# enricobottazzi/zk-fhe

Measured on AMD Instinct MI355X. Metric: BFV proofs/sec (k=13), higher is better.
Workload: dtype u32x8 (256-bit Montgomery integers over BN254 Fr/Fq)

## Files before the change

### zk-fhe_amd/csrc/core.hip

```cpp
#include <atomic>
#include <cstdio>
#include <cstdlib>
#include <cstring>

#include <map>
#include <mutex>
#include <utility>

#include "ctx.hpp"
#include "fq29.hip.hpp"
#include "fr29.hip.hpp"
#include "fr9.hip.hpp"

using namespace zk;

static thread_local std::string g_create_err;

int zk_fail(zkfhe_ctx *ctx, int code, const char *what, hipError_t e, const char *file, int line) {
  char buf[512];
  snprintf(buf, sizeof(buf), "%s failed: %s (%s:%d)", what, hipGetErrorString(e), file, line);
  if (ctx) ctx->err = buf; else g_create_err = buf;
  return code;
}
int zk_fail_msg(zkfhe_ctx *ctx, int code, const std::string &msg) {
// ... 11 lines not shown
  have = bytes;
  return ZKFHE_OK;
}

int zk_scratch(zkfhe_ctx *ctx, int slot, size_t bytes, void **out) {
  if (ctx->scratch_sz[slot] < bytes) {
    if (ctx->scratch[slot]) {
      ZK_HIP(ctx, hipStreamSynchronize(ctx->stream));
      ZK_HIP(ctx, hipFree(ctx->scratch[slot]));
      ctx->scratch[slot] = nullptr;
      ctx->scratch_sz[slot] = 0;
    }
    size_t want = bytes + bytes / 4;
    ZK_HIP(ctx, hipMalloc(&ctx->scratch[slot], want));
    ctx->scratch_sz[slot] = want;
  }
  *out = ctx->scratch[slot];
  return ZKFHE_OK;
}

Fr zk_fr_from_u64(uint64_t v) {
  Fr t = Fr::zero();
  t.l[0] = (u32)v;
  t.l[1] = (u32)(v >> 32);
  return fp_to_mont<FrP>(t);
}

Fr zk_fr_root_of_unity(int log_n) {
  Fr c;
  const u32 w[8] = {0x60c37c9cu, 0xd34f1ed9u, 0xd39329c8u, 0x3215cf6du, 0x3dd31f74u, 0x98865ea9u, 0x166d18b7u, 0x03ddb9f5u};
  for (int i = 0; i < 8; ++i) c.l[i] = w[i];
  Fr r = fp_to_mont<FrP>(c);
  for (int i = 0; i < 28 - log_n; ++i) r = fp_sqr<FrP>(r);
  return r;
}

__global__ void __launch_bounds__(256) k_copy16(const uint4 *__restrict__ src, uint4 *__restrict__ dst, size_t n16) {
  for (size_t i = blockIdx.x * (size_t)blockDim.x + threadIdx.x; i < n16; i += (size_t)gridDim.x * blockDim.x) dst[i] = src[i];
}
int zk_copy_d2d(zkfhe_ctx *ctx, void *dst, const void *src, size_t bytes) {
  if (!bytes) return ZKFHE_OK;
  if (bytes >= ((size_t)1 << 20) && (bytes & 15) == 0 && ((uintptr_t)dst & 15) == 0 && ((uintptr_t)src & 15) == 0) {
    const size_t n16 = bytes / 16;
    size_t blocks = (n16 + 255) / 256;
    const size_t cap = (size_t)ctx->num_cu * 32;
    k_copy16<<<(unsigned)(blocks > cap ? cap : blocks), 256, 0, ctx->stream>>>((const uint4 *)src, (uint4 *)dst, n16);
    ZK_LAUNCH_CHECK(ctx);
    return ZKFHE_OK;
  }
  ZK_HIP(ctx, zk_memcpy_async(ctx, dst, src, bytes, hipMemcpyDeviceToDevice, ctx->stream));
  return ZKFHE_OK;
}

extern "C" {

const char *zkfhe_version(void) { return "zkfhe-mi355x 0.1 (gfx950)"; }

int zkfhe_ctx_create(int device_id, void *hip_stream, zkfhe_ctx **out) {
  setenv("GPU_MAX_HW_QUEUES", "2", 0);
  if (!getenv("ZKFHE_SPIN_WAIT")) {
    (void)hipSetDevice(device_id);
    (void)hipSetDeviceFlags(hipDeviceScheduleBlockingSync);
    (void)hipGetLastError();
  }
  if (!out) return zk_fail_msg(nullptr, ZKFHE_EINVAL, "out is NULL");
  *out = nullptr;
  int count = 0;
  hipError_t e = hipGetDeviceCount(&count);
  if (e != hipSuccess || count == 0)
    return zk_fail_msg(nullptr, ZKFHE_ENODEV, std::string("no HIP device: ") + hipGetErrorString(e));
  if (device_id < 0 || device_id >= count) return zk_fail_msg(nullptr, ZKFHE_EINVAL, "device_id out of range");
  hipDeviceProp_t prop;
  ZK_HIP(nullptr, hipGetDeviceProperties(&prop, device_id));
  if (strncmp(prop.gcnArchName, "gfx950", 6) != 0)
    return zk_fail_msg(nullptr, ZKFHE_ENODEV, std::string("device is ") + prop.gcnArchName + ", this library is built for gfx950 only");
  ZK_HIP(nullptr, hipSetDevice(device_id));
  zkfhe_ctx *ctx = new zkfhe_ctx();
  static std::atomic<uint64_t> next_uid{1};
  ctx->uid = next_uid.fetch_add(1);
  ctx->device = device_id;
  ctx->num_cu = prop.multiProcessorCount;
  const char *chain_env = getenv("ZKFHE_CHAIN");
  ctx->chain_serial = chain_env && !strcmp(chain_env, "serial");
  const char *profile_env = getenv("ZKFHE_PROFILE");
  ctx->throughput = profile_env && !strcmp(profile_env, "throughput");
  if (hip_stream) {
    ctx->stream = (hipStream_t)hip_stream;
  } else {
    e = hipStreamCreateWithFlags(&ctx->stream, hipStreamNonBlocking);
    if (e != hipSuccess) { delete ctx; return zk_fail(nullptr, ZKFHE_EHIP, "hipStreamCreate", e, __FILE__, __LINE__); }
    ctx->own_stream = true;
  }
  if (hipHostMalloc(&ctx->bounce, zkfhe_ctx::BOUNCE_BYTES, hipHostMallocDefault) != hipSuccess) ctx->bounce = nullptr;
  if (hipEventCreateWithFlags(&ctx->wait_ev, hipEventBlockingSync | hipEventDisableTiming) != hipSuccess) ctx->wait_ev = nullptr;
  hipEventCreate(&ctx->ev0);
  hipEventCreate(&ctx->ev1);
  hipEventCreate(&ctx->pe0);
  hipEventCreate(&ctx->pe1);
  *out = ctx;
  return ZKFHE_OK;
}

int zkfhe_ctx_destroy(zkfhe_ctx *ctx) {
  ZK_ENTER(ctx);
  if (!ctx) return ZKFHE_OK;
  hipSetDevice(ctx->device);
  hipStreamSynchronize(ctx->stream);
  if (ctx->bounce) (void)hipHostFree(ctx->bounce);
  for (auto &kv : ctx->domains) {
    hipFree(kv.second.fwd);
    hipFree(kv.second.inv);
    hipFree(kv.second.fwd29);
    hipFree(kv.second.inv29);
    hipFree(kv.second.n_inv29_dev);
  }
  for (auto &kv : ctx->tw13) hipFree(kv.second);
  for (auto &kv : ctx->pre13) hipFree(kv.second);
  for (auto &kv : ctx->dif8) hipFree(kv.second);
  for (int i = 0; i < 4; ++i)
    if (ctx->scratch[i]) hipFree(ctx->scratch[i]);
  if (ctx->tickets) hipFree(ctx->tickets);
  if (ctx->bfv_tw) hipFree(ctx->bfv_tw);
  if (ctx->bfv_work) hipFree(ctx->bfv_work);
  for (auto &kv : ctx->slot_tw) hipFree(kv.second.dev);
  if (ctx->wait_ev) hipEventDestroy(ctx->wait_ev);
  hipEventDestroy(ctx->ev0);
  hipEventDestroy(ctx->ev1);
  if (ctx->own_stream) hipStreamDestroy(ctx->stream);
  delete ctx;
  return ZKFHE_OK;
}

const char *zkfhe_last_error(const zkfhe_ctx *ctx) { return ctx ? ctx->err.c_str() : g_create_err.c_str(); }

int zkfhe_sync(zkfhe_ctx *ctx) {
  ZK_ENTER(ctx);
  ZK_HIP(ctx, zk_wait(ctx));
  return ZKFHE_OK;
}

void *zkfhe_stream(zkfhe_ctx *ctx) { return (void *)ctx->stream; }

int zkfhe_device_info(zkfhe_ctx *ctx, char *arch_name, size_t arch_len, int *num_cu, size_t *hbm_bytes) {
  ZK_ENTER(ctx);
  hipDeviceProp_t prop;
  ZK_HIP(ctx, hipGetDeviceProperties(&prop, ctx->device));
  if (arch_name && arch_len) { strncpy(arch_name, prop.gcnArchName, arch_len - 1); arch_name[arch_len - 1] = 0; }
  if (num_cu) *num_cu = prop.multiProcessorCount;
  if (hbm_bytes) *hbm_bytes = prop.totalGlobalMem;
  return ZKFHE_OK;
}

int zkfhe_dev_alloc(zkfhe_ctx *ctx, size_t bytes, void **dptr) {
  ZK_ENTER(ctx);
  ZK_ARG(ctx, dptr != nullptr);
  ZK_HIP(ctx, hipSetDevice(ctx->device));
  hipError_t e = hipMalloc(dptr, bytes ? bytes : 1);
  if (e == hipErrorOutOfMemory) return zk_fail_msg(ctx, ZKFHE_ENOMEM, "hipMalloc: out of device memory");
  ZK_HIP(ctx, e);
  return ZKFHE_OK;
}
int zkfhe_dev_free(zkfhe_ctx *ctx, void *dptr) {
  ZK_ENTER(ctx);
  if (!dptr) return ZKFHE_OK;
  if (!ctx) {
    (void)hipFree(dptr);
// ... 300 lines not shown
```

### zk-fhe_amd/csrc/ctx.hpp

```cpp
#pragma once
#include <hip/hip_runtime.h>

#include <array>
#include <map>
#include <string>
#include <vector>

#include "../../include/zkfhe.h"
#include "bn254.hip.hpp"

struct NttDomain {
  int log_n = 0;
  zk::Fr *fwd = nullptr;
  zk::Fr *inv = nullptr;
  zk::Fr n_inv;
  zk::Fr omega, omega_inv;
  zk::Fr *fwd29 = nullptr, *inv29 = nullptr;
  zk::Fr n_inv29;
  zk::Fr *n_inv29_dev = nullptr;
};

struct zkfhe_ctx {
  uint64_t uid = 0;
  int device = 0;
  hipStream_t stream = nullptr;
  bool own_stream = false;
  hipEvent_t ev0 = nullptr, ev1 = nullptr;
  std::string err;
  int num_cu = 0;
  std::map<int, NttDomain> domains;
  std::map<const void *, void *> tw13;
  std::map<std::array<uint64_t, 6>, void *> pre13;
  std::map<std::array<uint64_t, 8>, void *> dif8;
  bool prof_on = false;
  hipEvent_t pe0 = nullptr, pe1 = nullptr;
  hipEvent_t wait_ev = nullptr;
  static constexpr int PROF_SLOTS = 28;
  double prof_ms[PROF_SLOTS] = {}, prof_bytes[PROF_SLOTS] = {}, prof_ops[PROF_SLOTS] = {};
  uint64_t prof_launches[PROF_SLOTS] = {};
  void *bounce = nullptr;
  static constexpr size_t BOUNCE_BYTES = (size_t)1 << 20;
  void *scratch[4] = {nullptr, nullptr, nullptr, nullptr};
  size_t scratch_sz[4] = {0, 0, 0, 0};
  float proof_marks[3] = {0, 0, 0};
  uint64_t cmd_count[3] = {0, 0, 0};
  zkfhe_ctx *cmd_owner = nullptr;
  bool chain_serial = false;
  bool throughput = false;
  unsigned *tickets = nullptr;
  uint32_t *bfv_tw = nullptr;
  void *bfv_work = nullptr;
  size_t bfv_work_sz = 0;
  struct SlotTables {
    uint32_t *dev = nullptr;
    uint32_t pinv = 0, n_inv = 0;
  };
  std::map<std::pair<uint64_t, uint64_t>, SlotTables> slot_tw;
};

struct zkfhe_basis {
  size_t n = 0;
  int c = 0;
  int windows = 0;
  zk::G1Affine *table = nullptr;
  zk::G1Affine *mult = nullptr;
  int mc = 0, mw = 0;
  size_t mult_bytes = 0;
  bool narrowed = false;
};

int zk_fail(zkfhe_ctx *ctx, int code, const char *what, hipError_t e, const char *file, int line);
int zk_fail_msg(zkfhe_ctx *ctx, int code, const std::string &msg);

#define ZK_HIP(ctx, expr)                                                             \
  do {                                                                                \
    hipError_t _e = (expr);                                                           \
    if (_e != hipSuccess) return zk_fail((ctx), ZKFHE_EHIP, #expr, _e, __FILE__, __LINE__); \
  } while (0)

enum { ZK_CMD_KERNEL = 0, ZK_CMD_COPY = 1, ZK_CMD_FILL = 2 };
static inline void zk_count(zkfhe_ctx *ctx, int which) { ++(ctx->cmd_owner ? ctx->cmd_owner : ctx)->cmd_count[which]; }

#define ZK_LAUNCH_CHECK(ctx)         \
  do {                               \
    zk_count((ctx), ZK_CMD_KERNEL);  \
    ZK_HIP(ctx, hipGetLastError());  \
  } while (0)

static inline hipError_t zk_memcpy_async(zkfhe_ctx *ctx, void *dst, const void *src, size_t bytes, hipMemcpyKind kind, hipStream_t stream) {
  zk_count(ctx, ZK_CMD_COPY);
  return hipMemcpyAsync(dst, src, bytes, kind, stream);
}
static inline hipError_t zk_memset_async(zkfhe_ctx *ctx, void *dst, int value, size_t bytes, hipStream_t stream) {
  zk_count(ctx, ZK_CMD_FILL);
  return hipMemsetAsync(dst, value, bytes, stream);
}

#define ZK_ENTER(ctx)                                   \
  do {                                                  \
    if (ctx) (void)hipSetDevice((ctx)->device);         \
  } while (0)

#define ZK_ARG(ctx, cond)                                                        \
  do {                                                                           \
    if (!(cond)) return zk_fail_msg((ctx), ZKFHE_EINVAL, std::string("bad argument: ") + #cond); \
  } while (0)

inline void zk_prof_begin(zkfhe_ctx *ctx) {
  if (ctx->prof_on) (void)hipEventRecord(ctx->pe0, ctx->stream);
}
inline void zk_prof_end(zkfhe_ctx *ctx, int which, double bytes) {
  if (!ctx->prof_on) return;
  (void)hipEventRecord(ctx->pe1, ctx->stream);
  (void)hipEventSynchronize(ctx->pe1);
  float ms = 0;
  (void)hipEventElapsedTime(&ms, ctx->pe0, ctx->pe1);
  ctx->prof_ms[which] += ms;
  ctx->prof_bytes[which] += bytes;
  ctx->prof_launches[which] += 1;
}

inline hipError_t zk_wait(zkfhe_ctx *ctx) {
  static const bool spin = getenv("ZKFHE_SPIN_WAIT") != nullptr;
  if (spin || !ctx->wait_ev) return hipStreamSynchronize(ctx->stream);
  hipError_t e = hipEventRecord(ctx->wait_ev, ctx->stream);
  if (e != hipSuccess) return e;
  return hipEventSynchronize(ctx->wait_ev);
}

int zk_dif8_pass(zkfhe_ctx *ctx, const zk::Fr *src, zk::Fr *dst, size_t n_cols, int log_n, int S, int inverse, const zk::Fr *shifts_host, unsigned rows);
int zk_msm_batch_strided(zkfhe_ctx *ctx, const zkfhe_basis *basis, const zkfhe_fr *scalars_dev, size_t col_stride, size_t n_cols, zkfhe_g1_affine *out_dev);
int zk_msm_batch_strided_form(zkfhe_ctx *ctx, const zkfhe_basis *basis, const zkfhe_fr *scalars_dev, size_t col_stride, size_t n_cols, void *out_dev, bool xyzz);
// ... 21 lines not shown
```

### zk-fhe_amd/csrc/msm.hip

```cpp
#include <algorithm>
#include <cstdio>
#include <cstring>
#include <vector>

#include "ctx.hpp"
#include "msm_plan.hpp"
#include "msm_sort.hip.hpp"
#include "msm_bucket.hip.hpp"
#include "msm_table.hip.hpp"

using namespace zk;

namespace {

constexpr size_t MSM_MAX_COLS = 4096;

__global__ void __launch_bounds__(256) k_g1_add(const G1Affine *__restrict__ a, const G1Affine *__restrict__ b,
                                                G1Affine *__restrict__ out, size_t n) {
  const size_t i = blockIdx.x * (size_t)blockDim.x + threadIdx.x;
  if (i >= n) return;
  G1X acc = g1x_from_affine(a[i]);
  g1x_add_affine(acc, b[i], false);
  out[i] = g1x_to_affine(acc);
}

__global__ void __launch_bounds__(256) k_g1_mul(const G1Affine *__restrict__ p, const Fr *__restrict__ k,
                                                G1Affine *__restrict__ out, size_t n) {
  const size_t i = blockIdx.x * (size_t)blockDim.x + threadIdx.x;
  if (i >= n) return;
  const Fr s = fp_from_mont<FrP>(k[i]);
  const G1Affine base = p[i];
  G1X acc = G1X::identity();
  for (int bit = 255; bit >= 0; --bit) {
    acc = g1x_dbl(acc);
    if ((s.l[bit >> 5] >> (bit & 31)) & 1) g1x_add_affine(acc, base, false);
  }
  out[i] = g1x_to_affine(acc);
}

int table_bits(size_t n, double budget_scale) {
  const char *e = getenv("ZKFHE_TABLE_BITS");
  const int forced = e ? atoi(e) : -1;
  const char *g = getenv("ZKFHE_TABLE_GB");
  double gb = g ? atof(g) : 48.0;
  if (!g) {
    size_t free_b = 0, total_b = 0;
    if (hipMemGetInfo(&free_b, &total_b) == hipSuccess && (double)free_b / 4.0 < gb * 1073741824.0) gb = (double)free_b / 4.0 / 1073741824.0;
  }
  const double budget = gb * 1073741824.0 * budget_scale;
  auto fits = [&](int c) {
    const double entries = (double)n * (double)((255 + c - 1) / c) * (double)(1u << (c - 1));
    return c >= 8 && c <= 15 && entries * sizeof(G1Affine) <= budget;
  };
  if (forced >= 0) return forced > 0 && fits(forced) ? forced : 0;
  for (int c = 15; c >= 8; --c)
    if (fits(c)) return c;
  return 0;
}

size_t table_reserve_bytes(size_t total_b) {
  if (const char *r = getenv("ZKFHE_TABLE_RESERVE_GB")) return (size_t)(atof(r) * 1073741824.0);
  const size_t eighth = total_b / 8, floor_b = (size_t)24 << 30;
  return eighth > floor_b ? eighth : floor_b;
}

BiasArg table_bias(int c, int W) {
  BiasArg B;
  memset(&B, 0, sizeof(B));
  for (int w = 0; w < W; ++w) {
    const int bit = c * w + c - 1;
    B.l[bit >> 5] |= 1u << (bit & 31);
  }
  return B;
}

int msm_table(zkfhe_ctx *ctx, const zkfhe_basis *basis, const Fr *scalars, size_t col_stride, size_t n_cols, void *out, bool xyzz) {
  const size_t n = basis->n;
  const int c = basis->mc, W = basis->mw;
  const size_t words = 2 * MSM_MAX_COLS + 4;
  if (!ctx->tickets) {
    ZK_HIP(ctx, hipMalloc((void **)&ctx->tickets, words * sizeof(unsigned)));
    ZK_HIP(ctx, zk_memset_async(ctx, ctx->tickets, 0, words * sizeof(unsigned), ctx->stream));
  }
  unsigned *n_part = ctx->tickets, *col_next = ctx->tickets + MSM_MAX_COLS;
  unsigned long long *adds = (unsigned long long *)(ctx->tickets + 2 * MSM_MAX_COLS);
  const size_t grid_max = (size_t)ctx->num_cu * 3;
#ifndef ZK_MSM_THROUGHPUT_P
#define ZK_MSM_THROUGHPUT_P 256
#endif
  size_t P = 256;
  const size_t P_min = ctx->throughput ? ZK_MSM_THROUGHPUT_P : 128;
  while (P > P_min && n_cols * ((n + P - 1) / P) < grid_max) P >>= 1;
  const size_t cpc = (n + P - 1) / P, n_items = n_cols * cpc;
  const size_t grid = n_items < grid_max ? n_items : grid_max;
  const size_t max_part = cpc < grid ? cpc : grid;
  const bool tree = n_cols <= 16;
  const unsigned L = tree ? 1 : 256;
  void *p0, *p1;
  ZK_CK(zk_scratch(ctx, 0, n_cols * max_part * L * sizeof(G1X), &p0));
  ZK_CK(zk_scratch(ctx, 1, grid * P * (size_t)W * 4, &p1));
  const int slot = n_cols * n > ((size_t)1 << 16) ? 0 : 2;
  if (ctx->prof_on) ZK_HIP(ctx, zk_memset_async(ctx, adds, 0, 8, ctx->stream));
  zk_prof_begin(ctx);
  (tree ? k_msm_table<true> : k_msm_table<false>)<<<(unsigned)grid, 256, 0, ctx->stream>>>(scalars, col_stride, n, basis->mult, c, W, table_bias(c, W), (unsigned)P, (unsigned)cpc,
                                                                                           (unsigned)n_cols, (unsigned)max_part, (G1X *)p0, n_part, col_next, (unsigned *)p1,
                                                                                           ctx->prof_on ? adds : nullptr);
  ZK_LAUNCH_CHECK(ctx);
  zk_prof_end(ctx, slot, 96.0 * (double)n * (double)n_cols);
  (xyzz ? k_msm_table_fold<true> : k_msm_table_fold<false>)<<<(unsigned)n_cols, 512, 0, ctx->stream>>>((const G1X *)p0, (unsigned)max_part, L, n_part, col_next, out);
  ZK_LAUNCH_CHECK(ctx);
  if (ctx->prof_on) {
    unsigned long long h = 0;
    ZK_HIP(ctx, hipMemcpy(&h, adds, 8, hipMemcpyDeviceToHost));
    ctx->prof_ops[slot] += (double)h;
  }
  return ZKFHE_OK;
}

int default_window_bits(size_t n) {
  if (n <= 64) return 5;
  if (n <= 1024) return 8;
  if (n <= 4096) return 11;
  if (n <= 16384) return 13;
  if (n <= 131072) return 14;
  return 16;
}

bool table_wide(const zkfhe_basis *b) {
  static const char *env = getenv("ZKFHE_TABLE_WIDE");
  return env ? env[0] == '1' : b->mw <= b->windows + 2;
}

static_assert(sizeof(G1X) == MSM_POINT_BYTES, "msm_plan.hpp sizes buckets, partials and marginals as G1X");
struct MsmScratch {
  char *p[MSM_ARRAYS];
  template <class T = unsigned>
  T *at(MsmArray a) const { return (T *)p[a]; }
};

int msm_scratch(zkfhe_ctx *ctx, const MsmGeometry &g, MsmScratch &a) {
  const MsmLayout l = msm_layout(g);
  void *slot[3];
  for (int s : {1, 2, 0}) ZK_CK(zk_scratch(ctx, s, l.slot_bytes[s], &slot[s]));
  for (int i = 0; i < MSM_ARRAYS; ++i) a.p[i] = (char *)slot[l.at[i].slot] + l.at[i].off;
  return ZKFHE_OK;
}

int sort_one_pass(zkfhe_ctx *ctx, const MsmGeometry &g, const MsmScratch &a, const Fr *scalars, size_t col_stride) {
  const unsigned gc = std::min(zk_blocks(g.n_cols * g.K1, 256), (unsigned)ctx->num_cu * 8);
  k_msm_clear<<<gc, 256, 0, ctx->stream>>>(a.at(HIST), g.n_cols * g.K1, a.at(HEAVY_COUNT));
  ZK_LAUNCH_CHECK(ctx);
  const unsigned chunks_per_col = (unsigned)((g.n + SORT_CHUNK - 1) / SORT_CHUNK);
  const unsigned grid = (unsigned)(g.n_cols * chunks_per_col);
  const size_t sort_lds = (size_t)g.K1 * sizeof(unsigned);
  if (sort_lds > 48 * 1024) {
    ZK_CK(zk_func_max_lds(ctx, (const void *)k_msm_hist, 160 * 1024));
    ZK_CK(zk_func_max_lds(ctx, (const void *)k_msm_scatter, 160 * 1024));
  }
  k_msm_hist<<<grid, SORT_THREADS, sort_lds, ctx->stream>>>(scalars, col_stride, g.n, chunks_per_col, g.c, g.W, a.at(HIST), g.K1);
  ZK_LAUNCH_CHECK(ctx);
  k_msm_scan<<<(unsigned)g.n_cols, 256, 0, ctx->stream>>>(a.at(HIST), a.at(OFF), a.at(CURSOR), g.K1);
  ZK_LAUNCH_CHECK(ctx);
  k_msm_scatter<<<grid, SORT_THREADS, sort_lds, ctx->stream>>>(scalars, col_stride, g.n, chunks_per_col, g.c, g.W, a.at(CURSOR), g.K1, a.at(ENTRIES), g.col_entries);
  ZK_LAUNCH_CHECK(ctx);
  return ZKFHE_OK;
}

int sort_two_level(zkfhe_ctx *ctx, const MsmGeometry &g, const MsmScratch &a, const Fr *scalars, size_t col_stride) {
  k_msm_clear<<<zk_blocks(g.n_cols * g.NB, 256), 256, 0, ctx->stream>>>(a.at(CHIST), g.n_cols * g.NB, a.at(HEAVY_COUNT));
  ZK_LAUNCH_CHECK(ctx);
  const unsigned ch_chunks = (unsigned)((g.n + CH_SCALARS - 1) / CH_SCALARS), cs_chunks = (unsigned)((g.n + CS_SCALARS - 1) / CS_SCALARS);
  k_msm_chist<<<(unsigned)(g.n_cols * ch_chunks), CS_THREADS, g.NB * sizeof(unsigned), ctx->stream>>>(scalars, col_stride, g.n, ch_chunks, g.c, g.W, g.L, g.NB, a.at(CHIST));
  ZK_LAUNCH_CHECK(ctx);
  k_msm_cscan<<<zk_blocks(g.n_cols, 64), 64, 0, ctx->stream>>>(a.at(CHIST), g.NB, g.n_cols, a.at(COFF), a.at(CCURSOR));
  ZK_LAUNCH_CHECK(ctx);
  const size_t cs_lds = ((size_t)3 * g.NB + (size_t)CS_SCALARS * g.W) * sizeof(unsigned);
  if (cs_lds > 48 * 1024) ZK_CK(zk_func_max_lds(ctx, (const void *)k_msm_cscatter, 64 * 1024));
  k_msm_cscatter<<<(unsigned)(g.n_cols * cs_chunks), CS_THREADS, cs_lds, ctx->stream>>>(scalars, col_stride, g.n, cs_chunks, g.c, g.W, g.L, g.NB, a.at(CCURSOR), a.at(STAGE),
                                                                                         g.stage_stride);
  ZK_LAUNCH_CHECK(ctx);
  ZK_CK(zk_func_max_lds(ctx, (const void *)k_msm_fine, (int)(FINE_TILE * sizeof(unsigned))));
  k_msm_fine<<<(unsigned)(g.n_cols * g.NB), FINE_THREADS, FINE_TILE * sizeof(unsigned), ctx->stream>>>(a.at(COFF), g.NB, g.L, a.at(STAGE), g.stage_stride, g.col_entries, g.K1,
                                                                                                        a.at(OFF), a.at(ENTRIES));
  ZK_LAUNCH_CHECK(ctx);
  return ZKFHE_OK;
}

int task_list(zkfhe_ctx *ctx, const MsmGeometry &g, const MsmScratch &a) {
  k_msm_task_count<<<(unsigned)g.n_cols, 256, 0, ctx->stream>>>(a.at(OFF), g.K, g.TASK_E, a.at(COL_HIST));
  ZK_LAUNCH_CHECK(ctx);
  k_msm_task_colscan<<<1, 128, 0, ctx->stream>>>(a.at(COL_HIST), (unsigned)g.n_cols, a.at(COL_BASE), a.at(N_TASKS));
  ZK_LAUNCH_CHECK(ctx);
  k_msm_task_fill<<<(unsigned)g.n_cols, 256, 0, ctx->stream>>>(a.at(OFF), g.K, g.TASK_E, a.at(COL_BASE), a.at(BUCKET_POS_A), a.at(BUCKET_POS_B), a.at<uint2>(TASKS),
// ... 216 lines not shown
```

### zk-fhe_amd/csrc/msm_table.hip.hpp

```cpp
#pragma once
#include "ctx.hpp"
#include "g1x29_wave.hip.hpp"

namespace {
using namespace zk;

struct BiasArg {
  u32 l[9];
};

__device__ __forceinline__ u32 bits_at(const u32 (&l)[9], int bit, int c) {
  const int limb = bit >> 5, sh = bit & 31;
  u32 lo = 0, hi = 0;
#pragma unroll
  for (int k = 0; k < 9; ++k) {
    if (k == limb) lo = l[k];
    if (k == limb + 1) hi = l[k];
  }
  return (u32)((((u64)hi << 32) | lo) >> sh) & ((1u << c) - 1);
}

__device__ __forceinline__ bool biased_scalar(const Fr &mont, const BiasArg &B, u32 (&out)[9], int &bits) {
  Fr s = fp_from_mont<FrP>(mont);
  const bool neg = fr_gt_half(s);
  if (neg) s = fp_neg<FrP>(s);
  bits = 0;
#pragma unroll
  for (int k = 0; k < 8; ++k)
    if (s.l[k]) bits = 32 * k + 32 - __clz(s.l[k]);
  u32 carry = 0;
#pragma unroll
  for (int k = 0; k < 8; ++k) {
    const u64 v = (u64)s.l[k] + B.l[k] + carry;
    out[k] = (u32)v;
    carry = (u32)(v >> 32);
  }
  out[8] = B.l[8] + carry;
  return neg;
}

__global__ void __launch_bounds__(64) k_basis_multiples(const G1Affine *__restrict__ bases, size_t n, int c, int W, G1Affine *__restrict__ T) {
  const size_t t = blockIdx.x * (size_t)blockDim.x + threadIdx.x;
  if (t >= n * (size_t)W) return;
  const size_t i = t / (size_t)W;
  const int w = (int)(t % (size_t)W);
  const size_t J = (size_t)1 << (c - 1);
  G1Affine *row = T + t * J;
  G1Affine b = bases[i];
  if (!b.is_identity() && w) b = g1x_to_affine(g1x_mul_pow2(g1x_from_affine(b), c * w));
  if (b.is_identity()) {
    for (size_t j = 0; j < J; ++j) row[j] = b;
    return;
  }
  row[0] = g1_affine_to_29(b);
  if (J == 1) return;
  G1X acc = g1x_from_affine_dbl(b);
  row[1] = g1_affine_to_29(g1x_to_affine(acc));
  for (size_t j = 2; j < J; ++j) {
    g1x_add_affine(acc, b, false);
    row[j] = g1_affine_to_29(g1x_to_affine(acc));
  }
}

template <bool TREE>
__global__ void __launch_bounds__(256, TREE ? 1 : 3) k_msm_table(const Fr *__restrict__ scalars, size_t col_stride, size_t n, const G1Affine *__restrict__ T, int c, int W, BiasArg B,
                                                   unsigned P, unsigned cpc , unsigned n_cols, unsigned max_part,
                                                   G1X *__restrict__ partials ,
                                                   unsigned *__restrict__ n_part ,
                                                   unsigned *__restrict__ col_next ,
                                                   unsigned *__restrict__ lists , unsigned long long *__restrict__ adds) {
  unsigned *__restrict__ lst = lists + (size_t)blockIdx.x * P * (unsigned)W;
  __shared__ G1X sh[TREE ? 128 : 1];
  __shared__ unsigned wave_cnt[4], item_sh;
  const unsigned lane = threadIdx.x & 63, wv = threadIdx.x >> 6;
  const int half = 1 << (c - 1);
  G1X29 acc = G1X29::identity();
  unsigned col = (unsigned)(((unsigned long long)blockIdx.x * n_cols) / gridDim.x), done = 0, total = 0;
  for (;;) {
    __syncthreads();
    if (threadIdx.x == 0) item_sh = atomicAdd(&col_next[col], 1u);
    __syncthreads();
    const unsigned chunk = item_sh;
    if (chunk >= cpc) {
      if (done) {
        if (TREE) acc = block_sum_256(acc, sh);
        __syncthreads();
        if (threadIdx.x == 0) item_sh = atomicAdd(&n_part[col], 1u);
        __syncthreads();
        const size_t slot = (size_t)col * max_part + item_sh;
        if (TREE) {
          if (threadIdx.x == 0) partials[slot] = g1x29_store(acc);
        } else {
          partials[slot * 256 + threadIdx.x] = g1x29_store(acc);
        }
        acc = G1X29::identity();
        done = 0;
      }
      __syncthreads();
      if (threadIdx.x == 0) item_sh = 0;
      __syncthreads();
      const unsigned MIN_JOIN = cpc < 4u ? cpc : 4u;
      unsigned best = 0;
      for (unsigned j = threadIdx.x; j < n_cols; j += 256) {
        const unsigned nx = __hip_atomic_load(&col_next[j], __ATOMIC_RELAXED, __HIP_MEMORY_SCOPE_AGENT);
        if (nx < cpc && (nx == 0 || cpc - nx >= MIN_JOIN)) {
          const unsigned h = ((j * 2654435761u) ^ (blockIdx.x * 40503u + 12345u) * 2246822519u) >> 13;
          best = max(best, (((h & 0x7ffffu) + 1u) << 12) | j);
        }
      }
      if (best) atomicMax(&item_sh, best);
      __syncthreads();
      const unsigned found = item_sh;
      if (!found) break;
      col = found & 4095u;
      continue;
    }
    ++done;
    {
      const size_t i = (size_t)chunk * P + threadIdx.x;
      const bool valid = threadIdx.x < P && i < n;
      u32 sb[9];
      bool neg = false;
      unsigned long long mask = 0;
      if (valid) {
        int bits;
        neg = biased_scalar(scalars[(size_t)col * col_stride + i], B, sb, bits);
        const int wtop = min(W, bits / c + 2);
        for (int w = 0; w < wtop; ++w)
          if ((int)bits_at(sb, w * c, c) != half) mask |= 1ull << w;
      }
      const unsigned mine = (unsigned)__popcll(mask);
      unsigned incl = mine;
#pragma unroll
      for (int d = 1; d < 64; d <<= 1) {
        const unsigned t = __shfl_up(incl, d);
        if ((int)lane >= d) incl += t;
      }
      if (lane == 63) wave_cnt[wv] = incl;
      __syncthreads();
      unsigned off = incl - mine;
      for (unsigned v = 0; v < wv; ++v) off += wave_cnt[v];
      const unsigned row0 = threadIdx.x * (unsigned)W;
      while (mask) {
        const int w = __builtin_ctzll(mask);
        mask &= mask - 1;
        const int d = (int)bits_at(sb, w * c, c) - half;
        lst[off++] = (((row0 + (unsigned)w) << (c - 1)) + (unsigned)(d < 0 ? -d : d) - 1u) | ((neg != (d < 0)) ? 0x80000000u : 0u);
      }
    }
    __syncthreads();
    const unsigned M = wave_cnt[0] + wave_cnt[1] + wave_cnt[2] + wave_cnt[3];
    total += M;
    const G1Affine *__restrict__ Tc = T + (((size_t)chunk * P * (size_t)W) << (c - 1));
    unsigned e = threadIdx.x, en = 0, en2 = 0;
    G1Affine p;
    if (e < M) {
      en = lst[e];
      p = Tc[en & 0x7fffffffu];
    }
    if (e + 256 < M) en2 = lst[e + 256];
    while (e < M) {
      const unsigned e2 = e + 256;
      unsigned en3 = 0;
      G1Affine p2;
      if (e2 < M) p2 = Tc[en2 & 0x7fffffffu];
      if (e2 + 256 < M) en3 = lst[e2 + 256];
      g1x29_add_affine(acc, g1a29_load(p), (en >> 31) != 0);
      e = e2;
      en = en2;
      en2 = en3;
      p = p2;
    }
  }
  if (adds && threadIdx.x == 0 && total) atomicAdd(adds, (unsigned long long)total);
}

template <bool XYZZ>
__global__ void __launch_bounds__(512) k_msm_table_fold(const G1X *__restrict__ partials, unsigned max_part, unsigned L, unsigned *__restrict__ n_part,
                                                        unsigned *__restrict__ col_next, void *__restrict__ out) {
  __shared__ G1X sh[256];
  const unsigned col = blockIdx.x, t = threadIdx.x & 255u, q = threadIdx.x >> 8;
  const unsigned np = n_part[col] * L;
  const G1X *mine = partials + (size_t)col * max_part * L;
  G1X29 f = G1X29::identity();
  {
    const unsigned first = L == 256 ? q * 256u + t : threadIdx.x, step = 512u;
    unsigned b = first;
    G1X cur;
    if (b < np) cur = mine[b];
    while (b < np) {
      const unsigned nb = b + step;
      G1X nxt;
      if (nb < np) nxt = mine[nb];
      g1x29_add(f, g1x29_load(cur));
      cur = nxt;
      b = nb;
    }
  }
  if (q == 1) sh[t] = g1x29_store(f);
  __syncthreads();
  if (q == 0) g1x29_add(f, g1x29_load(sh[t]));
  __syncthreads();
  if (q == 0 && t >= 128) sh[t - 128] = g1x29_store(f);
  __syncthreads();
  if (q == 0 && t < 128) g1x29_add(f, g1x29_load(sh[t]));
  __syncthreads();
  if (q == 0 && t >= 64 && t < 128) sh[t - 64] = g1x29_store(f);
  __syncthreads();
  if (threadIdx.x < 64) {
    g1x29_add(f, g1x29_load(sh[t]));
    for (int m = 1; m < 64; m <<= 1) {
      const G1X29 other = g1x_shfl_xor(f, m);
      g1x29_add(f, other);
    }
    if (threadIdx.x == 0) {
      if (XYZZ) ((G1X *)out)[col] = g1x29_to_std(f);
      else ((G1Affine *)out)[col] = g1x_to_affine(g1x29_to_std(f));
      n_part[col] = 0;
      col_next[col] = 0;
    }
  }
}

__global__ void __launch_bounds__(256) k_basis_table(const G1Affine *__restrict__ bases, size_t n, int c, int windows,
                                                     G1Affine *__restrict__ table) {
  const size_t i = blockIdx.x * (size_t)blockDim.x + threadIdx.x;
  if (i >= n) return;
  G1Affine p = bases[i];
  table[i] = g1_affine_to_29(p);
  G1X cur = g1x_from_affine(p);
  for (int w = 1; w < windows; ++w) {
    cur = g1x_mul_pow2(cur, c);
    G1Affine a = g1x_to_affine(cur);
    table[(size_t)w * n + i] = g1_affine_to_29(a);
    cur = g1x_from_affine(a);
  }
}

template <bool XYZZ>
__global__ void __launch_bounds__(64) k_msm_sparse(const zkfhe_sparse_term *__restrict__ terms, unsigned n_terms, const G1Affine *__restrict__ T, int c, int W,
                                                   BiasArg B, void *__restrict__ out) {
  const unsigned slot = blockIdx.x, lane = threadIdx.x;
  const int half = 1 << (c - 1);
  G1X29 acc = G1X29::identity();
  for (unsigned t = 0; t < n_terms; ++t) {
    if (terms[t].slot != slot) continue;
    Fr s;
#pragma unroll
    for (int i = 0; i < 4; ++i) {
      s.l[2 * i] = (u32)terms[t].scalar.l[i];
      s.l[2 * i + 1] = (u32)(terms[t].scalar.l[i] >> 32);
    }
    u32 sb[9];
    int bits;
    const bool neg = biased_scalar(s, B, sb, bits);
    const int d = (int)lane < W ? (int)bits_at(sb, (int)lane * c, c) - half : 0;
    if (d) {
// ... 16 lines not shown
```

### zk-fhe_amd/host/prove.hip

```cpp
#include "prover_internal.hpp"

int alloc_witness_buffers(zkfhe_ctx *ctx, const zkfhe_bfv_pk *pk, Workspace *ws) {
  if (ws->stream.p) return ZKFHE_OK;
  const size_t N = pk->prm.N;
  CK(ws->stream.alloc(ctx, (pk->gate1_cells + 8) * 32));
  CK(ws->pool.alloc(ctx, 40 * (2 * N + 8) * 32));
  CK(ws->invtmp.alloc(ctx, (pk->n_inv_slots + 8) * 32));
  ZK_HIP(ctx, hipHostMalloc((void **)&ws->host_pool, 24 * (2 * N + 8) * 32, hipHostMallocDefault));
  ws->host_poly_len = 2 * N + 8;
  ZK_HIP(ctx, hipHostMalloc((void **)&ws->host_poly, ws->host_poly_len * 32, hipHostMallocDefault));
  CK(ws->wblind.alloc(ctx, 256));
  ZK_HIP(ctx, hipHostMalloc((void **)&ws->ring, Workspace::RING_BYTES, hipHostMallocDefault));
  CK(ws->dev_ring.alloc(ctx, Workspace::RING_BYTES));
  {
    const CircuitConfig &c = pk->cfg;
    const size_t max_items = (size_t)c.n_advice() + c.n_fixed() + 2 + c.n_perm() + c.n_chunks() + 3 * c.n_lookup;
    ws->out_pts_cap = std::max<size_t>(ws->n_all, c.n_perm()) + 16;
    ws->out_ev_off = ws->out_pts_cap * PT_SLOT;
    ws->out_ev_cap = max_items * 4;
    ws->out_flag_off = ws->out_ev_off + ws->out_ev_cap * 32;
    ZK_HIP(ctx, hipHostMalloc((void **)&ws->host_out, ws->out_flag_off + 256, hipHostMallocDefault));
    memset(ws->host_out, 0, ws->out_flag_off + 256);
  }
  ZK_HIP(ctx, hipHostMalloc((void **)&ws->host_pts, ((size_t)pk->cfg.n_gate0 + 1) * PT_SLOT, hipHostMallocDefault));
// ... 467 lines not shown
zkp::Mat3 vandermonde3_inverse(const Fr c[3]) {
  zkp::Mat3 vinv;
  for (int k1 = 0; k1 < 3; ++k1) {
    const Fr &a = c[(k1 + 1) % 3], &b = c[(k1 + 2) % 3];
    const Fr den = fr_inv((c[k1] - a) * (c[k1] - b));
    vinv.v[0 * 3 + k1] = a * b * den;
    vinv.v[1 * 3 + k1] = (Fr::zero() - (a + b)) * den;
    vinv.v[2 * 3 + k1] = den;
  }
  return vinv;
}

void interpolate4(const Fr *pts, const Fr *vals, size_t np, Fr rc[4]) {
  for (int q = 0; q < 4; ++q) rc[q] = Fr::zero();
  for (size_t i = 0; i < np; ++i) {
    Fr num[4] = {Fr::one(), Fr::zero(), Fr::zero(), Fr::zero()};
    Fr den = Fr::one();
    size_t deg = 0;
    for (size_t t = 0; t < np; ++t) {
      if (t == i) continue;
      for (size_t q = ++deg; q > 0; --q) num[q] = num[q - 1] - pts[t] * num[q];
      num[0] = Fr::zero() - pts[t] * num[0];
      den = den * (pts[i] - pts[t]);
    }
    const Fr scl = vals[i] * fr_inv(den);
    for (size_t q = 0; q <= deg; ++q) rc[q] = rc[q] + num[q] * scl;
  }
}

void split_permuted(std::vector<AffinePoint> &pts, size_t n_adv, std::vector<AffinePoint> &permuted) {
  const size_t nl = (pts.size() - n_adv) / 2;
  permuted.resize(2 * nl);
  for (size_t i = 0; i < nl; ++i) permuted[2 * i] = pts[n_adv + i], permuted[2 * i + 1] = pts[n_adv + nl + i];
  pts.resize(n_adv);
}

struct Proof {
  zkfhe_ctx *const ctx;
  const zkfhe_srs *const srs;
  zkfhe_bfv_pk *const pk;
  const CircuitConfig &cfg;
  std::vector<U256> &instances;
  Trace &trace;
  Workspace *const ws;
  const NttDomain *const dom;
  const size_t n = cfg.n(), u = cfg.u(), nbl = n - u;
  const unsigned k = cfg.k;
  zkp::RngSeed rseed;
  const uint64_t ctr_adv = 0, ctr_lk = (uint64_t)cfg.n_advice() * nbl, ctr_pz = ctr_lk + 2 * (uint64_t)cfg.n_lookup * nbl,
                 ctr_lz = ctr_pz + (uint64_t)cfg.n_chunks() * (nbl - 1), ctr_rand = ctr_lz + (uint64_t)cfg.n_lookup * (nbl - 1);
  Transcript tr{cfg.transcript};
  bool host_witness = false, early_p1 = false, early_rand = false, inst_via_ring = false;
  const unsigned W_sh = srs->sharded() ? (unsigned)zkfhe_comm_world(srs->comm) : 1u, r_sh = srs->sharded() ? (unsigned)zkfhe_comm_rank(srs->comm) : 0u;
  const size_t c_lo = (size_t)cfg.n_chunks() * r_sh / W_sh, c_hi = (size_t)cfg.n_chunks() * (r_sh + 1) / W_sh;
  BfvState st;
  Assigner as{cfg, false, ws->host_adv};
  GpuPhase1 g1{ctx, pk, ws};
  std::vector<AffinePoint> permuted;
  U256 gamma_rlc;
  Fr beta, gamma, y, x;
  Fr *beta_delta_dev = nullptr;
  Fr pts_rot[6];
  std::vector<OpenItem> items;
  size_t idx_H = 0;
  double t_wit = 0;

  int rng_fill(hipStream_t stream, uint64_t ctr0, uint64_t ctr_col_stride, Fr *dst, size_t per_col, size_t col_stride, size_t n_cols) {
    if (!per_col || !n_cols) return ZKFHE_OK;
    zkp::k_rng_fill<<<grid_for(ctx, per_col * n_cols), 256, 0, stream>>>(rseed, ctr0, ctr_col_stride, dst, per_col, col_stride, n_cols);
    ZK_LAUNCH_CHECK(ctx);
    return ZKFHE_OK;
  }
  zkp::RngRows blind_rows(uint64_t ctr0, uint64_t ctr_col_stride) const {
    return zkp::RngRows{rseed, ctr0, ctr_col_stride, 1};
  }
  const zkfhe_basis *small_basis() const { return srs->g_lagrange_small ? srs->g_lagrange_small : srs->g_lagrange; }
  bool owns_chunk(size_t j) const { return j >= c_lo && j < c_hi; }
  bool owns_col(size_t perm_col) const { return owns_chunk(perm_col / cfg.chunk()); }
  int setup() {
    CK(zkfhe_sync(ctx));
    CK(alloc_witness_buffers(ctx, pk, ws));
    ws->aux->cmd_owner = ctx;
    ws->aux->throughput = ctx->throughput;
    ws->ring_off = ws->ring_flushed = 0;
    ws->inst_pending = false;
    trace.mark("setup (workspace)");
    early_rand = !srs->sharded();
    if (!early_rand) return ZKFHE_OK;
    zkfhe_ctx *aux = ws->aux;
    Fr *rand_c = ws->misc.fr() + 8 * n, *rand_l = ws->misc.fr() + 9 * n;
    CK(rng_fill(aux->stream, ctr_rand, 0, rand_c, n, n, 1));
    if (int rc = zkfhe_msm_batch_xyzz(aux, srs->g, (const zkfhe_fr *)rand_c, 1, (zkfhe_g1_xyzz *)ws->host_rand_pt))
      return zk_fail_msg(ctx, rc, std::string("random polynomial commitment (auxiliary stream): ") + zkfhe_last_error(aux));
    if (int rc = zkfhe_ntt_batch_to(aux, (const zkfhe_fr *)rand_c, (zkfhe_fr *)rand_l, 1, (int)k, 0))
      return zk_fail_msg(ctx, rc, std::string("random polynomial, Lagrange form (auxiliary stream): ") + zkfhe_last_error(aux));
    ZK_HIP(ctx, hipEventRecord(ws->ev_rand, aux->stream));
    return ZKFHE_OK;
  }
  int phase0(const char *input_json, const FastInput *words, std::vector<AffinePoint> &pts) {
    Context ctx0(CTX_PHASE0, false, false);
    std::vector<Cell> make_public;
    instances.clear();
    tr.common_scalar(pk->vk_digest);
    const auto on_public = [&](const std::vector<Cell> &pub) {
      instances.reserve(pub.size());
      for (const Cell &c : pub) instances.push_back(c.value);
      const size_t n_key = std::min<size_t>(instances.size(), 2 * (size_t)pk->prm.N);
      Transcript::State mid;
      if (input_json && pk->prehash.take(input_json, strlen(input_json), instances.data(), instances.size(), mid)) {
        tr.restore(mid);
      } else if (!n_key || !pk->prefix.capacity()) {
        tr.common_scalars_async(instances);
      } else if (pk->prefix.lookup(instances.data(), n_key, mid)) {
        tr.restore(mid);
        tr.common_scalars_async(std::vector<U256>(instances.begin() + (long)n_key, instances.end()));
      } else {
        PrefixCache *cache = &pk->prefix;
        std::vector<U256> key(instances.begin(), instances.begin() + (long)n_key);
        tr.common_scalars_async_marked(instances, n_key, [cache, key](const Transcript::State &st) { cache->insert(key.data(), key.size(), st); });
      }
    };
    std::string rendered;
    if (words ? !bfv_phase0_fast_values(ctx0, *words, pk->prm, make_public, st, on_public)
              : !bfv_phase0_fast(ctx0, input_json, strlen(input_json), pk->prm, make_public, st, on_public)) {
      if (words) {
        rendered = render_input_json(*words);
        input_json = rendered.c_str();
      }
      const CircuitInput in = CircuitInput::parse_json(input_json);
      trace.mark("parse_json");
      st = bfv_phase0(ctx0, in, pk->prm, make_public, on_public);
    }
    trace.mark("bfv_phase0");
    as.place(ctx0, true);
    trace.mark("place phase 0");
    if (instances.size() > n) return zk_fail_msg(ctx, ZKFHE_EINVAL, "more public inputs than rows");
    inst_via_ring = instances.size() * 32 <= ((size_t)1 << 20);
    if (inst_via_ring) {
      STAGE(staged, U256, ws, instances.data(), instances.size() * 32);
      ws->inst_src = (const Fr *)(ws->ring + ((const uint8_t *)staged - (const uint8_t *)ws->dev_ring.p));
      ws->inst_n = instances.size();
      ws->inst_pending = true;
    }
    trace.mark("transcript: instances");
    CK(blind_and_upload(0, cfg.n_gate0));
    trace.mark("blind + upload phase 0");
    const char *witness_env = getenv("ZKFHE_WITNESS");
    host_witness = witness_env && strcmp(witness_env, "host") == 0;
    const char *early_env = getenv("ZKFHE_EARLY_P1");
    const bool early_want = early_env ? early_env[0] == '1' : ((cfg.transcript == TR_POSEIDON && !ctx->throughput) || k >= 18);
    early_p1 = early_want && !host_witness && cfg.n_lookup > 0 && cfg.lookup_bits == 8;
    if (host_witness) return commit_cols(ctx, srs, small_basis(), ws->adv_l.fr(), cfg.n_gate0, (G1Affine *)ws->points.p, pts);
    CK(srs_msm_pts(ctx, srs, small_basis(), ws->adv_l.fr(), cfg.n_gate0, ws->host_pts));
    CK(srs_record(ctx, srs, ws->ev_pts));
    CK(g1.launch(st));
    if (early_p1) {
      CK(g1.place_early(blind_rows(ctr_adv + (uint64_t)cfg.n_gate0 * nbl, nbl), cfg.n_rlc));
      CK(permute_lookups(ws->host_early_err));
      CK(srs_msm_pts(ctx, srs, small_basis(), ws->adv_l.fr() + (size_t)cfg.n_gate0 * n, cfg.n_advice() - cfg.n_gate0 + 2 * cfg.n_lookup, ws->host_early));
      CK(srs_record(ctx, srs, ws->ev_early));
    }
    ZK_HIP(ctx, hipEventSynchronize(ws->ev_pts));
    pts.resize(cfg.n_gate0);
    points_canon(srs, ws->host_pts, cfg.n_gate0, pts.data());
    return ZKFHE_OK;
  }
// ... 867 lines not shown
```

Baseline: 277.0.

## Fuse MSM per-column fold into the table-sum kernel via last-block completion

Adds a fused variant of the table MSM kernel in which the block that completes a column's final chunk (detected with a per-column done counter) folds all of that column's partials and writes the output point. This removes the separate fold kernel launch and its serialization on the stream. The last exiting block resets the counters, so no host-side reset is needed. The trade-off is extra atomics and fence-based synchronization, plus a serial fold tail done by one block per column. The old two-kernel path stays available through an environment variable.

Result: no change. 275.2 (median of 2 runs) (-0.6%).

```diff
diff --git a/zk-fhe_amd/csrc/core.hip b/zk-fhe_amd/csrc/core.hip
--- a/zk-fhe_amd/csrc/core.hip
+++ b/zk-fhe_amd/csrc/core.hip
@@ -117,6 +117,8 @@
   ctx->num_cu = prop.multiProcessorCount;
   const char *chain_env = getenv("ZKFHE_CHAIN");
   ctx->chain_serial = chain_env && !strcmp(chain_env, "serial");
+  const char *fold_env = getenv("ZKFHE_MSM_FOLD");
+  ctx->msm_fold_separate = fold_env && !strcmp(fold_env, "separate");
   const char *profile_env = getenv("ZKFHE_PROFILE");
   ctx->throughput = profile_env && !strcmp(profile_env, "throughput");
   if (hip_stream) {
diff --git a/zk-fhe_amd/csrc/ctx.hpp b/zk-fhe_amd/csrc/ctx.hpp
--- a/zk-fhe_amd/csrc/ctx.hpp
+++ b/zk-fhe_amd/csrc/ctx.hpp
@@ -48,6 +48,7 @@
   bool chain_serial = false;
   bool throughput = false;
   unsigned *tickets = nullptr;
+  bool msm_fold_separate = false;
   uint32_t *bfv_tw = nullptr;
   void *bfv_work = nullptr;
   size_t bfv_work_sz = 0;
diff --git a/zk-fhe_amd/csrc/msm.hip b/zk-fhe_amd/csrc/msm.hip
--- a/zk-fhe_amd/csrc/msm.hip
+++ b/zk-fhe_amd/csrc/msm.hip
@@ -77,13 +77,14 @@
 int msm_table(zkfhe_ctx *ctx, const zkfhe_basis *basis, const Fr *scalars, size_t col_stride, size_t n_cols, void *out, bool xyzz) {
   const size_t n = basis->n;
   const int c = basis->mc, W = basis->mw;
-  const size_t words = 2 * MSM_MAX_COLS + 4;
+  const size_t words = 2 * MSM_MAX_COLS + 4 + MSM_MAX_COLS + 1;
   if (!ctx->tickets) {
     ZK_HIP(ctx, hipMalloc((void **)&ctx->tickets, words * sizeof(unsigned)));
     ZK_HIP(ctx, zk_memset_async(ctx, ctx->tickets, 0, words * sizeof(unsigned), ctx->stream));
   }
   unsigned *n_part = ctx->tickets, *col_next = ctx->tickets + MSM_MAX_COLS;
   unsigned long long *adds = (unsigned long long *)(ctx->tickets + 2 * MSM_MAX_COLS);
+  unsigned *col_done = ctx->tickets + 2 * MSM_MAX_COLS + 4, *exit_cnt = col_done + MSM_MAX_COLS;
   const size_t grid_max = (size_t)ctx->num_cu * 3;
 #ifndef ZK_MSM_THROUGHPUT_P
 #define ZK_MSM_THROUGHPUT_P 256
@@ -101,14 +102,23 @@
   ZK_CK(zk_scratch(ctx, 1, grid * P * (size_t)W * 4, &p1));
   const int slot = n_cols * n > ((size_t)1 << 16) ? 0 : 2;
   if (ctx->prof_on) ZK_HIP(ctx, zk_memset_async(ctx, adds, 0, 8, ctx->stream));
+  const BiasArg bias = table_bias(c, W);
+  unsigned long long *adds_arg = ctx->prof_on ? adds : nullptr;
   zk_prof_begin(ctx);
-  (tree ? k_msm_table<true> : k_msm_table<false>)<<<(unsigned)grid, 256, 0, ctx->stream>>>(scalars, col_stride, n, basis->mult, c, W, table_bias(c, W), (unsigned)P, (unsigned)cpc,
-                                                                                           (unsigned)n_cols, (unsigned)max_part, (G1X *)p0, n_part, col_next, (unsigned *)p1,
-                                                                                           ctx->prof_on ? adds : nullptr);
-  ZK_LAUNCH_CHECK(ctx);
-  zk_prof_end(ctx, slot, 96.0 * (double)n * (double)n_cols);
-  (xyzz ? k_msm_table_fold<true> : k_msm_table_fold<false>)<<<(unsigned)n_cols, 512, 0, ctx->stream>>>((const G1X *)p0, (unsigned)max_part, L, n_part, col_next, out);
-  ZK_LAUNCH_CHECK(ctx);
+  if (tree && !ctx->msm_fold_separate) {
+    (xyzz ? k_msm_table_fused<true> : k_msm_table_fused<false>)<<<(unsigned)grid, 256, 0, ctx->stream>>>(scalars, col_stride, n, basis->mult, c, W, bias, (unsigned)P, (unsigned)cpc,
+                                                                                                      (unsigned)n_cols, (unsigned)max_part, (G1X *)p0, n_part, col_next, (unsigned *)p1,
+                                                                                                      adds_arg, col_done, exit_cnt, out);
+    ZK_LAUNCH_CHECK(ctx);
+    zk_prof_end(ctx, slot, 96.0 * (double)n * (double)n_cols);
+  } else {
+    (tree ? k_msm_table<true> : k_msm_table<false>)<<<(unsigned)grid, 256, 0, ctx->stream>>>(scalars, col_stride, n, basis->mult, c, W, bias, (unsigned)P, (unsigned)cpc, (unsigned)n_cols,
+                                                                                             (unsigned)max_part, (G1X *)p0, n_part, col_next, (unsigned *)p1, adds_arg);
+    ZK_LAUNCH_CHECK(ctx);
+    zk_prof_end(ctx, slot, 96.0 * (double)n * (double)n_cols);
+    (xyzz ? k_msm_table_fold<true> : k_msm_table_fold<false>)<<<(unsigned)n_cols, 512, 0, ctx->stream>>>((const G1X *)p0, (unsigned)max_part, L, n_part, col_next, out);
+    ZK_LAUNCH_CHECK(ctx);
+  }
   if (ctx->prof_on) {
     unsigned long long h = 0;
     ZK_HIP(ctx, hipMemcpy(&h, adds, 8, hipMemcpyDeviceToHost));
diff --git a/zk-fhe_amd/csrc/msm_table.hip.hpp b/zk-fhe_amd/csrc/msm_table.hip.hpp
--- a/zk-fhe_amd/csrc/msm_table.hip.hpp
+++ b/zk-fhe_amd/csrc/msm_table.hip.hpp
@@ -62,6 +62,7 @@
   }
 }
 
+enum { FOLD_NONE = 0, FOLD_AFFINE = 1, FOLD_XYZZ = 2 };
 template <bool TREE>
 __global__ void __launch_bounds__(256, TREE ? 1 : 3) k_msm_table(const Fr *__restrict__ scalars, size_t col_stride, size_t n, const G1Affine *__restrict__ T, int c, int W, BiasArg B,
                                                    unsigned P, unsigned cpc , unsigned n_cols, unsigned max_part,
@@ -69,110 +70,21 @@
                                                    unsigned *__restrict__ n_part ,
                                                    unsigned *__restrict__ col_next ,
                                                    unsigned *__restrict__ lists , unsigned long long *__restrict__ adds) {
-  unsigned *__restrict__ lst = lists + (size_t)blockIdx.x * P * (unsigned)W;
-  __shared__ G1X sh[TREE ? 128 : 1];
-  __shared__ unsigned wave_cnt[4], item_sh;
-  const unsigned lane = threadIdx.x & 63, wv = threadIdx.x >> 6;
-  const int half = 1 << (c - 1);
-  G1X29 acc = G1X29::identity();
-  unsigned col = (unsigned)(((unsigned long long)blockIdx.x * n_cols) / gridDim.x), done = 0, total = 0;
-  for (;;) {
-    __syncthreads();
-    if (threadIdx.x == 0) item_sh = atomicAdd(&col_next[col], 1u);
-    __syncthreads();
-    const unsigned chunk = item_sh;
-    if (chunk >= cpc) {
-      if (done) {
-        if (TREE) acc = block_sum_256(acc, sh);
-        __syncthreads();
-        if (threadIdx.x == 0) item_sh = atomicAdd(&n_part[col], 1u);
-        __syncthreads();
-        const size_t slot = (size_t)col * max_part + item_sh;
-        if (TREE) {
-          if (threadIdx.x == 0) partials[slot] = g1x29_store(acc);
-        } else {
-          partials[slot * 256 + threadIdx.x] = g1x29_store(acc);
-        }
-        acc = G1X29::identity();
-        done = 0;
-      }
-      __syncthreads();
-      if (threadIdx.x == 0) item_sh = 0;
-      __syncthreads();
-      const unsigned MIN_JOIN = cpc < 4u ? cpc : 4u;
-      unsigned best = 0;
-      for (unsigned j = threadIdx.x; j < n_cols; j += 256) {
-        const unsigned nx = __hip_atomic_load(&col_next[j], __ATOMIC_RELAXED, __HIP_MEMORY_SCOPE_AGENT);
-        if (nx < cpc && (nx == 0 || cpc - nx >= MIN_JOIN)) {
-          const unsigned h = ((j * 2654435761u) ^ (blockIdx.x * 40503u + 12345u) * 2246822519u) >> 13;
-          best = max(best, (((h & 0x7ffffu) + 1u) << 12) | j);
-        }
-      }
-      if (best) atomicMax(&item_sh, best);
-      __syncthreads();
-      const unsigned found = item_sh;
-      if (!found) break;
-      col = found & 4095u;
-      continue;
-    }
-    ++done;
-    {
-      const size_t i = (size_t)chunk * P + threadIdx.x;
-      const bool valid = threadIdx.x < P && i < n;
-      u32 sb[9];
-      bool neg = false;
-      unsigned long long mask = 0;
-      if (valid) {
-        int bits;
-        neg = biased_scalar(scalars[(size_t)col * col_stride + i], B, sb, bits);
-        const int wtop = min(W, bits / c + 2);
-        for (int w = 0; w < wtop; ++w)
-          if ((int)bits_at(sb, w * c, c) != half) mask |= 1ull << w;
-      }
-      const unsigned mine = (unsigned)__popcll(mask);
-      unsigned incl = mine;
-#pragma unroll
-      for (int d = 1; d < 64; d <<= 1) {
-        const unsigned t = __shfl_up(incl, d);
-        if ((int)lane >= d) incl += t;
-      }
-      if (lane == 63) wave_cnt[wv] = incl;
-      __syncthreads();
-      unsigned off = incl - mine;
-      for (unsigned v = 0; v < wv; ++v) off += wave_cnt[v];
-      const unsigned row0 = threadIdx.x * (unsigned)W;
-      while (mask) {
-        const int w = __builtin_ctzll(mask);
-        mask &= mask - 1;
-        const int d = (int)bits_at(sb, w * c, c) - half;
-        lst[off++] = (((row0 + (unsigned)w) << (c - 1)) + (unsigned)(d < 0 ? -d : d) - 1u) | ((neg != (d < 0)) ? 0x80000000u : 0u);
-      }
-    }
-    __syncthreads();
-    const unsigned M = wave_cnt[0] + wave_cnt[1] + wave_cnt[2] + wave_cnt[3];
-    total += M;
-    const G1Affine *__restrict__ Tc = T + (((size_t)chunk * P * (size_t)W) << (c - 1));
-    unsigned e = threadIdx.x, en = 0, en2 = 0;
-    G1Affine p;
-    if (e < M) {
-      en = lst[e];
-      p = Tc[en & 0x7fffffffu];
-    }
-    if (e + 256 < M) en2 = lst[e + 256];
-    while (e < M) {
-      const unsigned e2 = e + 256;
-      unsigned en3 = 0;
-      G1Affine p2;
-      if (e2 < M) p2 = Tc[en2 & 0x7fffffffu];
-      if (e2 + 256 < M) en3 = lst[e2 + 256];
-      g1x29_add_affine(acc, g1a29_load(p), (en >> 31) != 0);
-      e = e2;
-      en = en2;
-      en2 = en3;
-      p = p2;
-    }
-  }
-  if (adds && threadIdx.x == 0 && total) atomicAdd(adds, (unsigned long long)total);
+  constexpr int FOLD = FOLD_NONE;
+  unsigned *const col_done = nullptr, *const exit_cnt = nullptr;
+  void *const out = nullptr;
+#include "msm_table_sum.inc"
+}
+
+template <bool XYZZ>
+__global__ void __launch_bounds__(256, 1) k_msm_table_fused(const Fr *__restrict__ scalars, size_t col_stride, size_t n, const G1Affine *__restrict__ T, int c, int W, BiasArg B,
+                                                            unsigned P, unsigned cpc, unsigned n_cols , unsigned max_part, G1X *__restrict__ partials ,
+                                                            unsigned *__restrict__ n_part, unsigned *__restrict__ col_next, unsigned *__restrict__ lists,
+                                                            unsigned long long *__restrict__ adds, unsigned *__restrict__ col_done ,
+                                                            unsigned *__restrict__ exit_cnt , void *__restrict__ out ) {
+  constexpr bool TREE = true;
+  constexpr int FOLD = XYZZ ? FOLD_XYZZ : FOLD_AFFINE;
+#include "msm_table_sum.inc"
 }
 
 template <bool XYZZ>
diff --git a/zk-fhe_amd/csrc/msm_table_sum.inc b/zk-fhe_amd/csrc/msm_table_sum.inc
--- /dev/null
+++ b/zk-fhe_amd/csrc/msm_table_sum.inc
@@ -0,0 +1,163 @@
+  static_assert(TREE || FOLD == FOLD_NONE, "the fold inside the launch sums one partial per visit");
+  unsigned *__restrict__ lst = lists + (size_t)blockIdx.x * P * (unsigned)W;
+  __shared__ G1X sh[TREE ? 128 : 1];
+  __shared__ unsigned wave_cnt[4], item_sh;
+  const unsigned lane = threadIdx.x & 63, wv = threadIdx.x >> 6;
+  const int half = 1 << (c - 1);
+  G1X29 acc = G1X29::identity();
+  unsigned col = (unsigned)(((unsigned long long)blockIdx.x * n_cols) / gridDim.x), done = 0, total = 0;
+  for (;;) {
+    __syncthreads();
+    if (threadIdx.x == 0) item_sh = atomicAdd(&col_next[col], 1u);
+    __syncthreads();
+    const unsigned chunk = item_sh;
+    if (chunk >= cpc) {
+      if (done) {
+        unsigned np = 0, folded = 0;
+        do {
+          if (TREE) acc = block_sum_256(acc, sh);
+          if (!np) {
+            __syncthreads();
+            if (threadIdx.x == 0) item_sh = atomicAdd(&n_part[col], 1u);
+            __syncthreads();
+            const size_t slot = (size_t)col * max_part + item_sh;
+            if (TREE && FOLD) {
+              if (threadIdx.x == 0) {
+                const G1X v = g1x29_store(acc);
+                const Fq *f[4] = {&v.x, &v.y, &v.zz, &v.zzz};
+                unsigned long long *dst = (unsigned long long *)&partials[slot];
+#pragma unroll
+                for (int i = 0; i < 16; ++i)
+                  __hip_atomic_store(dst + i, ((unsigned long long)f[i >> 2]->l[2 * (i & 3) + 1] << 32) | f[i >> 2]->l[2 * (i & 3)], __ATOMIC_RELAXED,
+                                     __HIP_MEMORY_SCOPE_AGENT);
+              }
+            } else if (TREE) {
+              if (threadIdx.x == 0) partials[slot] = g1x29_store(acc);
+            } else {
+              partials[slot * 256 + threadIdx.x] = g1x29_store(acc);
+            }
+            if (FOLD) {
+              __syncthreads();
+              if (threadIdx.x == 0) {
+                asm volatile("s_waitcnt vmcnt(0)" ::: "memory");
+                unsigned last = 0;
+                if (atomicAdd(&col_done[col], done) + done == cpc) {
+                  __builtin_amdgcn_fence(__ATOMIC_ACQUIRE, "agent");
+                  asm volatile("s_waitcnt vmcnt(0)" ::: "memory");
+                  last = __hip_atomic_load(&n_part[col], __ATOMIC_RELAXED, __HIP_MEMORY_SCOPE_AGENT);
+                }
+                item_sh = last;
+              }
+              __syncthreads();
+              np = item_sh;
+              if (np && threadIdx.x == 0) acc = G1X29::identity();
+            }
+          } else {
+            folded += 255;
+          }
+          if (FOLD && np) {
+            if (folded < np) {
+              const unsigned k = folded + threadIdx.x - 1u;
+              if (threadIdx.x) acc = k < np ? g1x29_load(partials[(size_t)col * max_part + k]) : G1X29::identity();
+            } else {
+              if (threadIdx.x == 0) {
+                if (FOLD == FOLD_XYZZ) ((G1X *)out)[col] = g1x29_to_std(acc);
+                else ((G1Affine *)out)[col] = g1x_to_affine(g1x29_to_std(acc));
+              }
+              np = 0;
+            }
+          }
+        } while (FOLD && np);
+        acc = G1X29::identity();
+        done = 0;
+      }
+      __syncthreads();
+      if (threadIdx.x == 0) item_sh = 0;
+      __syncthreads();
+      const unsigned MIN_JOIN = cpc < 4u ? cpc : 4u;
+      unsigned best = 0;
+      for (unsigned j = threadIdx.x; j < n_cols; j += 256) {
+        const unsigned nx = __hip_atomic_load(&col_next[j], __ATOMIC_RELAXED, __HIP_MEMORY_SCOPE_AGENT);
+        if (nx < cpc && (nx == 0 || cpc - nx >= MIN_JOIN)) {
+          const unsigned h = ((j * 2654435761u) ^ (blockIdx.x * 40503u + 12345u) * 2246822519u) >> 13;
+          best = max(best, (((h & 0x7ffffu) + 1u) << 12) | j);
+        }
+      }
+      if (best) atomicMax(&item_sh, best);
+      __syncthreads();
+      const unsigned found = item_sh;
+      if (!found) break;
+      col = found & 4095u;
+      continue;
+    }
+    ++done;
+    {
+      const size_t i = (size_t)chunk * P + threadIdx.x;
+      const bool valid = threadIdx.x < P && i < n;
+      u32 sb[9];
+      bool neg = false;
+      unsigned long long mask = 0;
+      if (valid) {
+        int bits;
+        neg = biased_scalar(scalars[(size_t)col * col_stride + i], B, sb, bits);
+        const int wtop = min(W, bits / c + 2);
+        for (int w = 0; w < wtop; ++w)
+          if ((int)bits_at(sb, w * c, c) != half) mask |= 1ull << w;
+      }
+      const unsigned mine = (unsigned)__popcll(mask);
+      unsigned incl = mine;
+#pragma unroll
+      for (int d = 1; d < 64; d <<= 1) {
+        const unsigned t = __shfl_up(incl, d);
+        if ((int)lane >= d) incl += t;
+      }
+      if (lane == 63) wave_cnt[wv] = incl;
+      __syncthreads();
+      unsigned off = incl - mine;
+      for (unsigned v = 0; v < wv; ++v) off += wave_cnt[v];
+      const unsigned row0 = threadIdx.x * (unsigned)W;
+      while (mask) {
+        const int w = __builtin_ctzll(mask);
+        mask &= mask - 1;
+        const int d = (int)bits_at(sb, w * c, c) - half;
+        lst[off++] = (((row0 + (unsigned)w) << (c - 1)) + (unsigned)(d < 0 ? -d : d) - 1u) | ((neg != (d < 0)) ? 0x80000000u : 0u);
+      }
+    }
+    __syncthreads();
+    const unsigned M = wave_cnt[0] + wave_cnt[1] + wave_cnt[2] + wave_cnt[3];
+    total += M;
+    const G1Affine *__restrict__ Tc = T + (((size_t)chunk * P * (size_t)W) << (c - 1));
+    unsigned e = threadIdx.x, en = 0, en2 = 0;
+    G1Affine p;
+    if (e < M) {
+      en = lst[e];
+      p = Tc[en & 0x7fffffffu];
+    }
+    if (e + 256 < M) en2 = lst[e + 256];
+    while (e < M) {
+      const unsigned e2 = e + 256;
+      unsigned en3 = 0;
+      G1Affine p2;
+      if (e2 < M) p2 = Tc[en2 & 0x7fffffffu];
+      if (e2 + 256 < M) en3 = lst[e2 + 256];
+      g1x29_add_affine(acc, g1a29_load(p), (en >> 31) != 0);
+      e = e2;
+      en = en2;
+      en2 = en3;
+      p = p2;
+    }
+  }
+  if (adds && threadIdx.x == 0 && total) atomicAdd(adds, (unsigned long long)total);
+  if (FOLD) {
+    __syncthreads();
+    if (threadIdx.x == 0) item_sh = atomicAdd(exit_cnt, 1u);
+    __syncthreads();
+    if (item_sh == gridDim.x - 1u) {
+      if (threadIdx.x < n_cols) {
+        __hip_atomic_store(&n_part[threadIdx.x], 0u, __ATOMIC_RELAXED, __HIP_MEMORY_SCOPE_AGENT);
+        __hip_atomic_store(&col_next[threadIdx.x], 0u, __ATOMIC_RELAXED, __HIP_MEMORY_SCOPE_AGENT);
+        __hip_atomic_store(&col_done[threadIdx.x], 0u, __ATOMIC_RELAXED, __HIP_MEMORY_SCOPE_AGENT);
+      }
+      if (threadIdx.x == 0) __hip_atomic_store(exit_cnt, 0u, __ATOMIC_RELAXED, __HIP_MEMORY_SCOPE_AGENT);
+    }
+  }
diff --git a/zk-fhe_amd/host/prove.hip b/zk-fhe_amd/host/prove.hip
--- a/zk-fhe_amd/host/prove.hip
+++ b/zk-fhe_amd/host/prove.hip
@@ -573,6 +573,7 @@
     CK(alloc_witness_buffers(ctx, pk, ws));
     ws->aux->cmd_owner = ctx;
     ws->aux->throughput = ctx->throughput;
+    ws->aux->msm_fold_separate = ctx->msm_fold_separate;
     ws->ring_off = ws->ring_flushed = 0;
     ws->inst_pending = false;
     trace.mark("setup (workspace)");
```
